# lazear/sage

Measured on NVIDIA H100. Metric: spectra/sec, higher is better.
Workload: dtype f32

## Files before the change

### sage_b200/csrc/kernels.cuh

```cuda
#pragma once
#include <type_traits>

#include "device_common.cuh"
#include "glibc_log.cuh"

#ifndef SAGE_B200_RARE_NOINLINE
#define SAGE_B200_RARE_NOINLINE 0
#endif
#if SAGE_B200_RARE_NOINLINE
#define SB_RARE __noinline__
#else
#define SB_RARE __forceinline__
#endif

namespace sb {

__device__ __forceinline__ uint32_t pep_partition(const DbView& db, float x, bool le) {
    uint32_t lo = 0, hi = db.n_pep;
    if (db.pep_lut != nullptr) {
        const float t = (x - db.plut_base) * db.plut_inv_w;
        if (t == t) {
            const int c = (int)fminf(fmaxf(floorf(t), -2.0f), (float)PEP_LUT_CELLS + 2.0f);
            lo = __ldg(db.pep_lut + min(max(c - 1, 0), (int)PEP_LUT_CELLS));
            hi = __ldg(db.pep_lut + min(max(c + 2, 0), (int)PEP_LUT_CELLS));
        }
    }
    const int kx = f32_key(x);
    while (lo < hi) {
        const uint32_t mid = lo + ((hi - lo) >> 1);
        const int k = f32_key(__ldg(db.pep_mono + mid));
        if (le ? k <= kx : k < kx) lo = mid + 1; else hi = mid;
    }
    return lo;
}

__global__ void k_setup_queries(DbView db, ScorerView sc, BatchView b, uint32_t* sort_key, uint32_t* sort_val) {
    __shared__ unsigned long long s_sum[4][8];
    const uint32_t s = blockIdx.x * blockDim.x + threadIdx.x;
    unsigned long long nq = 0, nwide = 0, maxpot = 0, npepq = 0, list_need = 0, ncta = 0;
    if (s < b.n) {
    const float pmz = b.prec_mz[s];
    const uint32_t known = b.prec_charge[s];
    const float mz = __fsub_rn(pmz, PROTON);
    const bool fold = sc.wide_window || !(known != 0 && !sc.override_charge);
    uint32_t c0 = fold ? sc.min_charge : known;
    uint32_t c1 = fold ? sc.max_charge : known;
    QueryDesc* out = b.queries + (size_t)s * sc.qmax;
    uint32_t qi = 0;
    for (uint32_t z = c0; z <= c1 && qi < sc.qmax; z++) {
        const float precursor_mass = __fmul_rn(mz, (float)z);
        Tol ptol = sc.precursor_tol;
        if (sc.wide_window) {
            float lo = -2.4f, hi = 2.4f;
            if (b.iso_lo != nullptr && !isnan(b.iso_lo[s]) && !isnan(b.iso_hi[s])) { lo = b.iso_lo[s]; hi = b.iso_hi[s]; }
            ptol.kind = 2;
            ptol.lo = __fmul_rn(lo, (float)z);
            ptol.hi = __fmul_rn(hi, (float)z);
        }
        const uint32_t mfc = max_fragment_charge(sc.max_fragment_charge_opt, z);
        for (uint32_t ii = 0; ii < sc.n_iso; ii++, qi++) {
            const int iso = (sc.min_iso != sc.max_iso) ? sc.min_iso + (int)ii : 0;
            const float qmass = __fsub_rn(precursor_mass, __fmul_rn((float)iso, NEUTRON));
            float plo, phi;
            tol_bounds(ptol, qmass, plo, phi);
            const uint32_t ppl = pep_partition(db, plo, false);
            const uint32_t left = ppl == 0 ? 0 : ppl - 1;
            const uint32_t right = max(left, pep_partition(db, phi, true));
            QueryDesc q;
            q.pre_lo = left;
            q.pre_hi = right;
            q.potential = right - left + 1;
            const bool lo_ok = left < db.n_pep && __ldg(db.pep_mono + left) >= plo;
            const bool hi_ok = right < db.n_pep && __ldg(db.pep_mono + right) <= phi;
            const long long elo = (long long)left + (lo_ok ? 0 : 1);
            const long long ehi = (long long)right - (hi_ok ? 0 : 1);
            if (ehi < elo) { q.eff_lo = 1; q.eff_hi = 0; } else { q.eff_lo = (uint32_t)elo; q.eff_hi = (uint32_t)ehi; }
            q.charge = (uint8_t)z;
            q.iso = (int8_t)iso;
            q.nfc = (uint8_t)(mfc - 1);
            q.mode = q.potential > NARROW_CAP ? 2 : ((db.pep_centric_ok && q.potential <= sc.pep_cap) ? 3 : (q.potential <= WARPQ_CAP ? 4 : 1));
            out[qi] = q;
            if (q.mode != 2 && q.potential > sc.kparam) list_need += q.potential;
            if (q.mode == 4) b.counters[C_COUNT + qi] = 1ull;
            ncta += (q.mode == 1 || q.mode == 3);
            nq++;
            if (q.mode == 2) {
                nwide++;
                QueryHits h0; h0.n = 0; h0.default_run = q.potential; h0.matched_peaks = 0; h0.scored_candidates = 0;
                b.hits[(size_t)s * sc.qmax + qi] = h0;
            }
            if (q.mode == 3) npepq++;
            if (q.potential > maxpot) maxpot = q.potential;
        }
    }
    for (; qi < sc.qmax; qi++) {
        QueryDesc q = {};
        out[qi] = q;
    }
    if (sort_key) { sort_key[s] = out[0].mode ? out[0].pre_lo : 0xFFFFFFFFu; sort_val[s] = s; }
    if (nwide) {
        unsigned long long w = atomicAdd(b.counters + C_WIDE, nwide);
        for (uint32_t j = 0; j < sc.qmax; j++)
            if (out[j].mode == 2) { if (w < b.wide_cap) b.wide_items[w] = s * sc.qmax + j; w++; }
    }
    if (ncta) {
        unsigned long long w = atomicAdd(b.counters + C_NCTA, ncta);
        for (uint32_t j = 0; j < sc.qmax; j++)
            if (out[j].mode == 1 || out[j].mode == 3) b.cta_items[w++] = s * sc.qmax + j;
    }
    for (uint32_t j = 0; j < sc.qmax; j++) {
        ReplaySlot rs; rs.off = 0; rs.item = s * sc.qmax + j; rs.n_list = 0; rs.state = 1; rs.k = 0;
        b.nslots[(size_t)s * sc.qmax + j] = rs;
    }
    }
    const uint32_t lane = threadIdx.x & 31, warp = threadIdx.x >> 5;
// ... 206 lines not shown
                        matched++;
                    }
                }
                if (stop) { e = cnt; break; }
            }
        }
        uint32_t pend = __ballot_sync(0xffffffffu, e < cnt);
        while (pend) {
            const int src = __ffs(pend) - 1;
            pend &= pend - 1;
            const uint32_t e0 = __shfl_sync(0xffffffffu, e, src);
            const float lo_s = __shfl_sync(0xffffffffu, flo, src), hi_s = __shfl_sync(0xffffffffu, fhi, src);
            for (uint32_t pos = e0; pos < cnt; pos += 32) {
                const uint32_t i = pos + lane;
                bool stop = i >= cnt;
                if (!stop) {
                    const float fmz = __ldg(mz + i);
                    const uint32_t pid = pep0 + __ldg(off + i);
                    stop = fmz > hi_s;
                    if (!stop && fmz >= lo_s) {
                        if (pid >= q.eff_lo && pid <= q.eff_hi) {
                            const uint32_t idx = pid - q.pre_lo;
                            atomicAdd(&cnt32[idx >> 1], 1u << ((idx & 1) * 16));
                            matched++;
                        }
                    }
                }
                if (__any_sync(0xffffffffu, stop)) break;
            }
        }
    }
}

__device__ __forceinline__ void narrow_cta_query(const DbView& db, const ScorerView& sc, const BatchView& b, uint32_t pmax, uint64_t* nlist, uint32_t item,
                                                 float* bounds_smem, const NarrowIndexView& nv) {
    __shared__ uint32_t cnt32[NARROW_CAP / 2 + 1];
    __shared__ uint32_t s_warp[40];
    ReplaySlot* const nslots = b.nslots;
    const uint32_t s = item / sc.qmax;
    const QueryDesc q = b.queries[item];
    const uint32_t tid = threadIdx.x, lane = tid & 31, warp = tid >> 5, nwarps = PRELIM_THREADS / 32;
    const uint32_t p0 = b.peak_off[s], np = b.peak_off[s + 1] - p0;
    const uint32_t nwords = (q.potential + 1) >> 1;
    for (uint32_t i = tid; i < nwords; i += PRELIM_THREADS) cnt32[i] = 0;
    __shared__ unsigned long long s_loff;
    if (tid == 0 && q.potential > sc.kparam) s_loff = atomicAdd(b.counters + C_NLIST, (unsigned long long)q.potential);

    const uint32_t nfc = q.nfc;
    const uint32_t ntask = np * nfc;
    uint32_t my_matched = 0, my_pages = 0, my_entries = 0;
    __shared__ LutParams s_lp[8];
    bool pep_path = q.mode == 3 && np > 0 && np < 65536 && nfc <= 8;
    float* const bnd = bounds_smem;
    uint16_t* const luts = reinterpret_cast<uint16_t*>(bounds_smem + 2 * (size_t)nfc * pmax);
    if (pep_path) {
        for (uint32_t t = tid; t < ntask; t += PRELIM_THREADS) {
            const uint32_t c = t / np, p = t - c * np;
            const float mass = __fmul_rn(__ldg(b.masses + p0 + p), (float)(c + 1));
            float flo, fhi;
            tol_bounds(sc.fragment_tol, mass, flo, fhi);
            bnd[(2 * c) * pmax + p] = flo;
            bnd[(2 * c + 1) * pmax + p] = fhi;
        }
        __syncthreads();
        bool bad = false;
        for (uint32_t t = tid; t < ntask; t += PRELIM_THREADS) {
            const uint32_t c = t / np, p = t - c * np;
            const float* lo_c = bnd + (2 * c) * pmax;
            const float* hi_c = lo_c + pmax;
            if (p > 0) bad |= !(lo_c[p] >= lo_c[p - 1]) || !(hi_c[p] >= hi_c[p - 1]);
            bad |= !(lo_c[p] == lo_c[p]) || !(hi_c[p] == hi_c[p]);
        }
        if (__syncthreads_or(bad)) {
            pep_path = false;
            if (tid == 0) atomicAdd(b.counters + C_PEPFALLBACK, 1ull);
        } else {
            for (uint32_t c = 0; c < nfc; c++) {
                const float* lo_c = bnd + (2 * c) * pmax;
                const float* hi_c = lo_c + pmax;
// ... 83 lines not shown
        for (uint32_t w = 0; w < nwarps; w++) { pages_total += s_red[1][w]; entries_total += s_red[2][w]; }
        atomicAdd(b.counters + C_TASKS, (unsigned long long)ntask);
        if (pages_total) atomicAdd(b.counters + C_PAGES, (unsigned long long)pages_total);
        if (entries_total) atomicAdd(b.counters + C_ENTRIES, (unsigned long long)entries_total);
        atomicAdd(b.counters + C_MATCHED, (unsigned long long)matched_total);
    }
    QueryHits* h = b.hits + item;
    if (matched_total == 0) {
        if (tid == 0) {
            h->n = 0; h->default_run = q.potential; h->matched_peaks = 0; h->scored_candidates = 0;
            nslots[item].off = 0; nslots[item].item = item; nslots[item].n_list = 0; nslots[item].state = 1; nslots[item].k = 0;
        }
        return;
    }
    const uint32_t n = q.potential, k = min(n, sc.kparam);
    auto cnt = [&](uint32_t i) -> uint32_t { return (cnt32[i >> 1] >> ((i & 1) * 16)) & 0xFFFFu; };
    ReplaySlot* slot = nslots + item;
    uint32_t nzc = 0;
    if (n <= k) {
        uint64_t* keys = b.hit_keys + (size_t)item * sc.kparam;
        for (uint32_t i = tid; i < n; i += PRELIM_THREADS) {
            const uint32_t c = cnt(i);
            nzc += c != 0;
            keys[i] = c ? prescore_key(c, q.pre_lo + i, q.charge, q.iso) : PRESCORE_DEFAULT;
        }
        const uint32_t nzt = block_sum_u32(nzc, s_warp);
        if (tid == 0) {
            h->n = n; h->default_run = 0; h->matched_peaks = matched_total; h->scored_candidates = nzt;
            slot->off = 0; slot->item = item; slot->n_list = 0; slot->state = 1; slot->k = k;
        }
        return;
    }
    const unsigned long long loff = s_loff;
    if (loff + n > b.nlist_cap) {
        if (tid == 0) {
            h->n = 0; h->default_run = q.potential; h->matched_peaks = 0; h->scored_candidates = 0;
            slot->off = 0; slot->item = item; slot->n_list = 0; slot->state = 1; slot->k = 0;
        }
        return;
    }
    uint64_t* list = nlist + loff;
    for (uint32_t i = tid; i < k; i += PRELIM_THREADS) {
        const uint32_t c = cnt(i);
        nzc += c != 0;
        list[i] = c ? prescore_key(c, q.pre_lo + i, q.charge, q.iso) : PRESCORE_DEFAULT;
    }
    uint32_t wbase = k;
    for (uint32_t base = k; base < n; base += PRELIM_THREADS) {
        const uint32_t i = base + tid;
        const uint32_t c = i < n ? cnt(i) : 0;
        nzc += c != 0;
        const uint32_t ball = __ballot_sync(0xffffffffu, c != 0);
        if (lane == 0) s_warp[warp] = __popc(ball);
        __syncthreads();
        uint32_t off = 0, total = 0;
        for (uint32_t w = 0; w < nwarps; w++) {
            const uint32_t x = s_warp[w];
            if (w < warp) off += x;
            total += x;
        }
        if (c) list[wbase + off + __popc(ball & ((1u << lane) - 1))] = prescore_key(c, q.pre_lo + i, q.charge, q.iso);
        wbase += total;
        __syncthreads();
    }
    const uint32_t nzt = block_sum_u32(nzc, s_warp);
    if (tid == 0) {
        h->n = k; h->default_run = 0; h->matched_peaks = matched_total; h->scored_candidates = nzt;
        slot->off = loff; slot->item = item; slot->n_list = wbase; slot->state = 0; slot->k = k;
    }
}

__global__ void __launch_bounds__(PRELIM_THREADS, PRELIM_CTAS) k_prelim_narrow(DbView db, ScorerView sc, BatchView b, uint32_t pmax, uint64_t* nlist, NarrowIndexView nv) {
    extern __shared__ float bounds_smem[];
    const uint32_t total = (uint32_t)min(b.counters[C_NCTA], (unsigned long long)b.n * sc.qmax);
    for (uint32_t i = blockIdx.x; i < total; i += gridDim.x) {
        narrow_cta_query(db, sc, b, pmax, nlist, b.cta_items[i], bounds_smem, nv);
        __syncthreads();
    }
}

template <bool BLK>
__global__ void __launch_bounds__(WARPQ_WARPS * 32, WARPQ_MIN_CTAS) k_prelim_narrow_warp(DbView db, ScorerView sc, BatchView b, uint64_t* nlist, uint32_t s_lo,
                                                                                                uint32_t s_hi, NarrowIndexView nv) {
    __shared__ uint32_t cnt_all[WARPQ_WARPS][WARPQ_CAP / 2];
    if (b.counters[C_COUNT + blockIdx.y] == 0ull) return;
    const uint32_t lane = threadIdx.x & 31, warp = threadIdx.x >> 5;
    const uint32_t pos = blockIdx.x * WARPQ_WARPS + warp;
    if (pos >= b.n) return;
    const uint32_t s = b.order ? b.order[pos] : pos;
    if (s < s_lo || s >= s_hi) return;
    const uint32_t item = s * sc.qmax + blockIdx.y;
    const QueryDesc q = b.queries[item];
    if (q.mode != 4) return;
    uint32_t* const cnt32 = cnt_all[warp];
    const uint32_t n = q.potential, k = min(n, sc.kparam);
    for (uint32_t i = lane; i < (n + 1) >> 1; i += 32) cnt32[i] = 0;
    unsigned long long loff = 0;
    if (n > k) {
        if (lane == 0) loff = atomicAdd(b.counters + C_NLIST, (unsigned long long)n);
        loff = __shfl_sync(0xffffffffu, loff, 0);
    }
    __syncwarp();
    const uint32_t p0 = b.peak_off[s], np = b.peak_off[s + 1] - p0;
    const uint32_t nfc = q.nfc, ntask = np * nfc;
    uint32_t matched = 0, pages = 0, entries = 0;
    const uint32_t blk0 = BLK ? q.pre_lo / nv.block : 0u, blk1 = BLK ? min(q.pre_hi, db.n_pep - 1) / nv.block : 0u;
    for (uint32_t t0 = 0; t0 < ntask; t0 += 32) {
        const uint32_t t = t0 + lane;
        const bool act = t < ntask;
        float flo = 0.0f, fhi = 0.0f;
        if (act) {
            const uint32_t p = t / nfc, fc = t - p * nfc + 1;
            const float mass = __fmul_rn(__ldg(b.masses + p0 + p), (float)fc);
            tol_bounds(sc.fragment_tol, mass, flo, fhi);
        }
        if (BLK) block_probe_warp(nv, q, blk0, blk1, act, flo, fhi, cnt32, matched);
        else if (act) index_probe(db, q, flo, fhi, cnt32, matched, pages, entries);
    }
    for (int o = 16; o > 0; o >>= 1) {
        matched += __shfl_xor_sync(0xffffffffu, matched, o);
        pages += __shfl_xor_sync(0xffffffffu, pages, o);
        entries += __shfl_xor_sync(0xffffffffu, entries, o);
    }
    __syncwarp();
    if (lane == 0) {
        atomicAdd(b.counters + C_TASKS, (unsigned long long)ntask);
        if (pages) atomicAdd(b.counters + C_PAGES, (unsigned long long)pages);
        if (entries) atomicAdd(b.counters + C_ENTRIES, (unsigned long long)entries);
        if (matched) atomicAdd(b.counters + C_MATCHED, (unsigned long long)matched);
    }
    QueryHits* h = b.hits + item;
    ReplaySlot* slot = b.nslots + item;
    if (matched == 0 || (n > k && loff + n > b.nlist_cap)) {
        if (lane == 0) { h->n = 0; h->default_run = n; h->matched_peaks = 0; h->scored_candidates = 0; }
        return;
    }
    auto cnt = [&](uint32_t i) -> uint32_t { return (cnt32[i >> 1] >> ((i & 1) * 16)) & 0xFFFFu; };
    uint32_t nzc = 0;
    uint64_t* dst = n <= k ? b.hit_keys + (size_t)item * sc.kparam : nlist + loff;
    for (uint32_t i = lane; i < k; i += 32) {
        const uint32_t c = cnt(i);
        nzc += c != 0;
        dst[i] = c ? prescore_key(c, q.pre_lo + i, q.charge, q.iso) : PRESCORE_DEFAULT;
    }
    uint32_t wbase = k;
    for (uint32_t base = k; base < n; base += 32) {
        const uint32_t i = base + lane;
        const uint32_t c = i < n ? cnt(i) : 0;
        nzc += c != 0;
        const uint32_t ball = __ballot_sync(0xffffffffu, c != 0);
        if (c) dst[wbase + __popc(ball & ((1u << lane) - 1))] = prescore_key(c, q.pre_lo + i, q.charge, q.iso);
        wbase += __popc(ball);
    }
    for (int o = 16; o > 0; o >>= 1) nzc += __shfl_xor_sync(0xffffffffu, nzc, o);
    if (lane == 0) {
        h->n = k; h->default_run = 0; h->matched_peaks = matched; h->scored_candidates = nzc;
        if (n > k) { slot->off = loff; slot->n_list = wbase; slot->state = 0; slot->k = k; }
    }
}

#ifndef SAGE_B200_WIDE_THREADS
#define SAGE_B200_WIDE_THREADS 512
#endif
#ifndef SAGE_B200_WIDE_TILE
#define SAGE_B200_WIDE_TILE (32 * 1024)
#endif
#ifndef SAGE_B200_WIDE_CTAS
#define SAGE_B200_WIDE_CTAS 2
#endif
constexpr int WIDE_THREADS = SAGE_B200_WIDE_THREADS;
constexpr int WIDE_CTAS = SAGE_B200_WIDE_CTAS;
constexpr bool WIDE_SMALL = WIDE_CTAS > 1;
constexpr uint32_t WIDE_TILE = SAGE_B200_WIDE_TILE;
constexpr uint32_t WIDE_VMAX = WIDE_SMALL ? 1024 : 2048;
constexpr uint32_t WIDE_TCACHE = WIDE_SMALL ? 1024 : 2048;
constexpr uint32_t WIDE_LMAX = 12288;
constexpr uint32_t WIDE_HLEV = 64;
typedef ReplaySlot WideSlot;
struct WideRange { uint64_t start; uint32_t len; float flo, fhi; };

constexpr uint32_t WIDE_VCAP = WIDE_SMALL ? 512 : 1024;
constexpr uint32_t WIDE_BT = 16;
struct WideSlow {
    uint32_t cur[WIDE_VMAX];
// ... 567 lines not shown
    const QueryDesc q = b.queries[item];
    const uint32_t s = item / sc.qmax;
    const uint32_t p0 = b.peak_off[s], np = b.peak_off[s + 1] - p0;
    const uint32_t nfc = q.nfc, ntask = np * nfc;
    if (ntask > WIDE_TMAX) return;
    unsigned long long pages = 0, entries = 0;
    for (uint32_t t = lane; t < ntask; t += 32) {
        const uint32_t p = t / nfc, fc = t - p * nfc + 1;
        const float mass = __fmul_rn(__ldg(b.masses + p0 + p), (float)fc);
        float flo, fhi;
        tol_bounds(sc.fragment_tol, mass, flo, fhi);
        uint32_t bl, br;
        bucket_range(db, flo, fhi, bl, br);
        for (uint32_t page = bl; page < br; page++) {
            const uint64_t pbase = (uint64_t)page * db.bucket_size;
            const uint32_t pn = (uint32_t)(min(pbase + db.bucket_size, db.n_frag) - pbase);
            const uint32_t st = page_lower_bound_dir(db, page, db.frag + pbase, pn, q.pre_lo);
            const uint32_t en = page_lower_bound_dir(db, page, db.frag + pbase, pn, q.pre_hi + 1);
            entries += en - (st == 0 ? 0 : st - 1);
            pages++;
        }
    }
    for (int o = 16; o > 0; o >>= 1) {
        pages += __shfl_down_sync(0xffffffffu, pages, o);
        entries += __shfl_down_sync(0xffffffffu, entries, o);
    }
    if (lane == 0) {
        if (pages) atomicAdd(b.counters + C_PAGES, pages);
        if (entries) atomicAdd(b.counters + C_ENTRIES, entries);
    }
}

constexpr int REPLAY_THREADS = 128;
template <bool COMPACT>
__global__ void __launch_bounds__(REPLAY_THREADS) k_replay(ScorerView sc, BatchView b, const uint64_t* lists, const ReplaySlot* slots, uint32_t n_slots,
                                                           const unsigned long long* n_slots_dev, uint32_t n_spectra) {
    typedef typename std::conditional<COMPACT, uint32_t, uint64_t>::type key_t;
    extern __shared__ __align__(8) unsigned char rheap_raw[];
    key_t* const rheap = reinterpret_cast<key_t*>(rheap_raw);
    uint32_t slot = blockIdx.x * REPLAY_THREADS + threadIdx.x;
    if (n_slots_dev != nullptr) n_slots = (uint32_t)min((unsigned long long)n_slots, *n_slots_dev);
    if (slot >= n_slots) return;
    if (n_spectra) { const uint32_t pos = slot % n_spectra; slot = (b.order ? b.order[pos] : pos) * sc.qmax + slot / n_spectra; }
    const ReplaySlot ws = slots[slot];
    if (ws.state != 0) return;
    const uint64_t* list = lists + ws.off;
    const uint32_t k = ws.k, tid = threadIdx.x;
    uint32_t pre_lo = 0, q_charge = 0;
    int q_iso = 0;
    if (COMPACT) { const QueryDesc q = b.queries[ws.item]; pre_lo = q.pre_lo; q_charge = q.charge; q_iso = q.iso; }
    auto pack = [&](uint64_t k64) -> key_t {
        if (!COMPACT) return (key_t)k64;
        return (key_t)(key_peptide(k64) == 0xFFFFFFFFu ? 0x0000FFFFu : ((key_matched(k64) << 16) | (key_peptide(k64) - pre_lo)));
    };
    auto unpack = [&](key_t kk) -> uint64_t {
        if (!COMPACT) return (uint64_t)kk;
        const uint32_t v = (uint32_t)kk;
        return v == 0x0000FFFFu ? PRESCORE_DEFAULT : prescore_key(v >> 16, pre_lo + (v & 0xFFFFu), q_charge, q_iso);
    };
    auto H = [&](uint32_t i) -> key_t& { return rheap[i * REPLAY_THREADS + tid]; };
    auto sift = [&](uint32_t index, key_t val) {
        for (;;) {
            const uint32_t l = index * 2 + 1;
            if (l >= k) break;
            uint32_t c = l;
            key_t cv = H(l);
            if (l + 1 < k) { const key_t cr = H(l + 1); if (cr < cv) { cv = cr; c = l + 1; } }
            if (!(cv < val)) break;
            H(index) = cv;
            index = c;
        }
        H(index) = val;
    };
    for (uint32_t i = 0; i < k; i++) H(i) = pack(__ldg(list + i));
    for (uint32_t i = k / 2; i-- > 0;) sift(i, H(i));
    key_t root = H(0);
    uint64_t nxt = k < ws.n_list ? __ldg(list + k) : 0;
    for (uint32_t j = k; j < ws.n_list; j++) {
        const key_t kq = pack(nxt);
        if (j + 1 < ws.n_list) nxt = __ldg(list + j + 1);
        if (kq > root) { sift(0, kq); root = H(0); }
    }
    uint64_t* keys = b.hit_keys + (size_t)ws.item * sc.kparam;
    for (uint32_t i = 0; i < k; i++) keys[i] = unpack(H(i));
}

struct ScoreRec {
    double hyperscore;
    uint32_t peptide;
    uint32_t matched_b, matched_y;
    float summed_b, summed_y;
    uint32_t longest_b, longest_y;
    float ppm_difference;
    uint32_t charge;
    int iso;
    uint32_t valid;
    uint32_t plen;
};

__device__ SB_RARE int select_most_intense_peak(const float* masses, const float* intens, uint32_t n, float center, const Tol& tol) {
    float lo, hi;
    tol_bounds(tol, center, lo, hi);
    lo = __fadd_rn(lo, 0.0f);
    hi = __fadd_rn(hi, 0.0f);
    const int klo = f32_key(lo), khi = f32_key(hi);
    uint32_t i, j;
    binary_search_slice(n, [&](uint32_t k) { return f32_key(masses[k]) < klo; }, [&](uint32_t k) { return f32_key(masses[k]) <= khi; }, i, j);
    int best = -1;
    float max_int = 0.0f;
    for (uint32_t idx = i; idx < j; idx++) {
        const float m = masses[idx];
        if (m >= lo && m <= hi) {
            const float it = intens[idx];
            if (it >= max_int) { max_int = it; best = (int)idx; }
        }
    }
    return best;
// ... 1350 lines not shown
```

### sage_b200/csrc/sage_b200.cu

```cuda
#include <cub/device/device_radix_sort.cuh>
#include <cub/device/device_scan.cuh>
#include <cub/device/device_select.cuh>
#include <cub/device/device_reduce.cuh>
#include <cuda_runtime.h>
#include <thrust/iterator/counting_iterator.h>

#include <pthread.h>
#include <sched.h>

#include <algorithm>
#include <atomic>
#include <cctype>
#include <cmath>
#include <cstdarg>
#include <cstdio>
#include <cstdlib>
#include <cstring>
#include <chrono>
#include <condition_variable>
#include <memory>
#include <mutex>
#include <thread>
#include <string>
#include <vector>
// ... 1147 lines not shown

    CUDA_TRY(cudaStreamWaitEvent(st, S->lanes[(&L - S->lanes) ^ 1].ev[4], 0));
    CUDA_TRY(cudaStreamWaitEvent(st, L.ev_small, 0));
    CUDA_TRY(cudaEventRecord(L.ev[6], st));
    CUDA_TRY(cudaMemsetAsync(L.d_counters.p, 0, 8 * (C_COUNT + (size_t)sv.qmax), st));
    const bool annotate = sv.annotate && S->frag_dst != nullptr;
    if (annotate) {
        if ((rc = L.d_frags.reserve(S->frag_cap * sizeof(sage_b200_fragment) + 64))) return rc;
        unsigned long long* hbase = (unsigned long long*)L.h_counters.p + C_COUNT + 1;
        *hbase = S->frag_used;
        CUDA_TRY(cudaMemcpyAsync(L.d_counters.as<unsigned long long>() + C_FRAGS, hbase, 8, cudaMemcpyHostToDevice, st));
    }
    ScorerView svq = sv;
    uint32_t mfc = sv.max_fragment_charge_opt >= 0 ? std::min<uint32_t>(C.zmax, (uint32_t)(sv.max_fragment_charge_opt + 1) & 0xFF) : C.zmax;
    if (mfc < 2) mfc = 2;
    size_t pep_smem = (size_t)(mfc - 1) * (2 * (size_t)C.pmax * sizeof(float) + 2 * LUT_CELLS * sizeof(uint16_t));
    if (mfc - 1 > 8) pep_smem = 200 * 1024;
    if (pep_smem > 96 * 1024) { svq.pep_cap = 0; pep_smem = 0; }
    if (svq.pep_cap == 0) pep_smem = 0;
    uint32_t *sk_in = nullptr, *sk_out = nullptr, *sv_in = nullptr, *sv_out = nullptr;
    int sort_bits = 1;
    while (sort_bits < 32 && (db->v.n_pep >> sort_bits)) sort_bits++;
    const int sort_lo = std::max(0, sort_bits - 16);
    size_t sort_tmp = 0;
    if (S->sort_spectra && n > 1) {
        if ((rc = L.d_sort.reserve(16 * (size_t)n))) return rc;
        sk_in = L.d_sort.as<uint32_t>(); sk_out = sk_in + n; sv_in = sk_out + n; sv_out = sv_in + n;
        CUDA_TRY(cub::DeviceRadixSort::SortPairs(nullptr, sort_tmp, sk_in, sk_out, sv_in, sv_out, (int)n, sort_lo, sort_bits, st));
        if ((rc = L.d_sorttmp.reserve(sort_tmp + 16))) return rc;
    }
    C.nlist_cap = std::max<uint64_t>(C.force_nlist, (uint64_t)std::ceil(S->nlist_per_spectrum * (double)n) + 4096);
    C.wide_cap = (uint32_t)std::min<uint64_t>(C.nitems, std::max<uint64_t>(C.force_wide, S->wide_per_spectrum > 0.0
                                                                               ? (uint64_t)std::ceil(S->wide_per_spectrum * 1.1 * (double)n) + 64 : 0));
    if ((rc = L.d_nlist.reserve(8 * (C.nlist_cap + 16)))) return rc;
    if ((rc = L.d_nslots.reserve(C.nitems * sizeof(ReplaySlot)))) return rc;
    if (C.wide_cap) {
        if ((rc = L.d_witems.reserve(4 * (size_t)C.wide_cap))) return rc;
        if ((rc = L.d_wlist.reserve((size_t)C.wide_cap * WIDE_LMAX * 8))) return rc;
        if ((rc = L.d_wslots.reserve((size_t)C.wide_cap * sizeof(WideSlot)))) return rc;
    }
    if ((rc = L.d_citems.reserve(4 * C.nitems))) return rc;
    bv.cta_items = L.d_citems.as<uint32_t>();
    bv.nslots = L.d_nslots.as<ReplaySlot>();
    bv.wide_items = L.d_witems.as<uint32_t>();
    bv.wide_cap = C.wide_cap;
    bv.nlist_cap = C.nlist_cap;
    k_setup_queries<<<(n + 127) / 128, 128, 0, st>>>(db->v, svq, bv, sk_in, sv_in);
    CUDA_TRY(cudaGetLastError());
    if (sk_in) {
        CUDA_TRY(cub::DeviceRadixSort::SortPairs(L.d_sorttmp.p, sort_tmp, sk_in, sk_out, sv_in, sv_out, (int)n, sort_lo, sort_bits, st));
        bv.order = sv_out;
    }
    CUDA_TRY(cudaEventRecord(L.ev[2], st));
    if (C.nparts <= 1) CUDA_TRY(cudaStreamWaitEvent(st, L.ev_masses, 0));
    uint64_t launches = 1;

    const size_t rsm = (size_t)sv.kparam * REPLAY_THREADS * 8;
    const float ptol_span = std::max(std::fabs(sv.precursor_tol.lo), std::fabs(sv.precursor_tol.hi));
    const bool narrow_tol = ptol_span <= (sv.precursor_tol.kind == 0 ? 2000.0f : sv.precursor_tol.kind == 1 ? 0.2f : 5.0f);
    NarrowIndexView nv{};
    if (S->narrow_index && !sv.wide_window && narrow_tol) {
        if (S->narrow_block == 0 && (rc = narrow_block_for(S))) return rc;
        nv = db_narrow_index(db, S->narrow_block ? S->narrow_block : S->narrow_block_auto, S->narrow_block != 0);
    }
    for (uint32_t q = 0; q < C.nparts; q++) {
        if (C.nparts > 1) CUDA_TRY(cudaStreamWaitEvent(st, L.ev_part[q], 0));
        const dim3 wgrid((n + WARPQ_WARPS - 1) / WARPQ_WARPS, sv.qmax);
        if (nv.mz != nullptr) k_prelim_narrow_warp<true><<<wgrid, WARPQ_WARPS * 32, 0, st>>>(db->v, svq, bv, L.d_nlist.as<uint64_t>(), C.part_lo[q], C.part_lo[q + 1], nv);
        else k_prelim_narrow_warp<false><<<wgrid, WARPQ_WARPS * 32, 0, st>>>(db->v, svq, bv, L.d_nlist.as<uint64_t>(), C.part_lo[q], C.part_lo[q + 1], nv);
        CUDA_TRY(cudaGetLastError());
        launches += q > 0;
    }
    if (C.nparts > 1) CUDA_TRY(cudaStreamWaitEvent(st, L.ev_masses, 0));
    k_prelim_narrow<<<(unsigned)std::min<uint64_t>(C.nitems, (uint64_t)db->sm_count * PRELIM_CTAS), PRELIM_THREADS, pep_smem, st>>>(db->v, svq, bv, C.pmax, L.d_nlist.as<uint64_t>(),
                                                                                                                         S->narrow_cta ? nv : NarrowIndexView{});
    CUDA_TRY(cudaGetLastError());
    CUDA_TRY(cudaEventRecord(L.ev[8], st));
    k_replay<true><<<(unsigned)((C.nitems + REPLAY_THREADS - 1) / REPLAY_THREADS), REPLAY_THREADS, rsm / 2, st>>>(sv, bv, L.d_nlist.as<uint64_t>(), L.d_nslots.as<ReplaySlot>(),
                                                                                                                 (uint32_t)C.nitems, nullptr, n);
    CUDA_TRY(cudaGetLastError());
    launches += 3;
    if (C.wide_cap) {
        const int ctas = (int)std::min<uint64_t>((uint64_t)db->sm_count * WIDE_CTAS, C.wide_cap);
        const WideIndexView wv = db_wide_index(db, sv.wide_tile);
        k_prelim_wide<<<ctas, WIDE_THREADS, sizeof(WideSmem), st>>>(db->v, sv, bv, (uint32_t)C.nitems, L.d_wlist.as<uint64_t>(), L.d_wslots.as<WideSlot>(), wv);
        CUDA_TRY(cudaGetLastError());
        if (wv.frag != nullptr) {
            k_wide_account<<<(C.wide_cap + 7) / 8, 256, 0, st>>>(db->v, sv, bv);
            CUDA_TRY(cudaGetLastError());
            launches++;
        }
        k_replay<false><<<(unsigned)((C.wide_cap + REPLAY_THREADS - 1) / REPLAY_THREADS), REPLAY_THREADS, rsm, st>>>(
            sv, bv, L.d_wlist.as<uint64_t>(), L.d_wslots.as<WideSlot>(), C.wide_cap, L.d_counters.as<unsigned long long>() + C_WIDE, 0u);
        CUDA_TRY(cudaGetLastError());
        launches += 2;
    }
    CUDA_TRY(cudaEventRecord(L.ev[3], st));

    if ((rc = lane_join_stager(L))) return rc;
    CUDA_TRY(cudaStreamWaitEvent(st, L.ev_intens, 0));
    const bool split = S->score_split && !sv.chimera && !annotate && !dbg && S->quick_mode == 0;
    if (split) {
        C.hits_cap = std::max<uint64_t>(C.force_hits, (uint64_t)std::ceil((S->hits_per_spectrum > 0.0 ? S->hits_per_spectrum : 4096.0) * (double)n) + 65536);
        if ((rc = L.d_cand.reserve((size_t)n * sv.kparam * sizeof(CandOut)))) return rc;
        if ((rc = L.d_meta.reserve((size_t)n * sizeof(SpecMeta)))) return rc;
        if ((rc = L.d_recs.reserve((size_t)n * sv.kparam * sizeof(ScoreRec)))) return rc;
        if ((rc = L.d_hkey.reserve((size_t)n * sv.kparam * 8))) return rc;
        if ((rc = L.d_emit.reserve((size_t)n * sv.report_psms * 4 + 16))) return rc;
        if ((rc = L.d_hitk.reserve(2 * C.hits_cap + 16))) return rc;
        if ((rc = L.d_hiti.reserve(4 * C.hits_cap + 16))) return rc;
        if ((rc = L.d_hitt.reserve(4 * C.hits_cap + 16))) return rc;
        SplitOut so{};
// ... 1748 lines not shown
        FDR_TRY(cudaGetLastError());
    }
    k_rt_align<<<(unsigned)((n_files + 127) / 128), 128, 0, st>>>(d_mat, d_mean, n_rows, n_files, d_maxrt, d_align);
    FDR_TRY(cudaGetLastError());
    float* d_aligned = d_out[0];
    k_rt_aligned<<<g, 256, 0, st>>>(d_rows, d_file, n, d_align, d_aligned);
    FDR_TRY(cudaGetLastError());
    FDR_TRY(cudaEventRecord(ev[2], st));

    if (int rc = rt_model<0>(st, A, fma, pk, d_rows, n, d_train, n_train, d_aligned, d_aligned, d_out[1], d_out[2], &out->rt_fitted, &out->rt_r2,
                             &out->rt_eps, out->rt_beta))
        return rc;
    FDR_TRY(cudaEventRecord(ev[3], st));
    if (int rc = rt_model<1>(st, A, fma, pk, d_rows, n, d_train, n_train, nullptr, d_aligned, d_out[3], d_out[4], &out->ims_fitted, &out->ims_r2,
                             &out->ims_eps, out->ims_beta))
        return rc;
    FDR_TRY(cudaEventRecord(ev[4], st));

    float* dst[5] = {out->aligned_rt, out->predicted_rt, out->delta_rt_model, out->predicted_ims, out->delta_ims_model};
    for (int c = 0; c < 5; c++) FDR_TRY(cudaMemcpyAsync(dst[c], d_out[c], 4 * n, cudaMemcpyDeviceToHost, st));
    if (out->spectrum_q) FDR_TRY(cudaMemcpyAsync(out->spectrum_q, d_q, 4 * n, cudaMemcpyDeviceToHost, st));
    FDR_TRY(cudaMemcpyAsync(out->alignments, d_align, sizeof(sage_b200_alignment) * n_files, cudaMemcpyDeviceToHost, st));
    FDR_TRY(cudaStreamSynchronize(st));
    out->training_rows = n_train;
    out->aligned_peptides = n_rows;
    float* ms[4] = {&out->ms_sort_q, &out->ms_alignment, &out->ms_rt_model, &out->ms_ims_model};
    for (int i = 0; i < 4; i++) FDR_TRY(cudaEventElapsedTime(ms[i], ev[i], ev[i + 1]));
    FDR_TRY(cudaEventElapsedTime(&out->ms_total, ev[0], ev[4]));
    return 0;
}
#undef FDR_TRY

#if SAGE_B200_PHASE_CLOCKS
extern "C" int sage_b200_debug_phase_cycles(unsigned long long* out16, int reset) {
    if (out16) CUDA_TRY(cudaMemcpyFromSymbol(out16, g_phase, sizeof(unsigned long long) * 16));
    if (reset) { unsigned long long z[16] = {0}; CUDA_TRY(cudaMemcpyToSymbol(g_phase, z, sizeof z)); }
    return 0;
}
#endif
```

Before: 24.73 million.

## Store narrow candidate lists as compact 32-bit keys and restructure replay heap

Narrow prelim kernels now write 32-bit compact keys (matched<<16 | offset) into the candidate list instead of 64-bit prescore keys. List reservations are padded to multiples of four so replay can fetch four keys per vector load. The replay kernel loads each heap cooperatively across the warp, keeps the top seven heap nodes in registers, uses a two-level sift, and writes outputs coalesced per warp. This halves list memory traffic and cuts shared-memory work per replacement, at the cost of more registers and more code complexity. It also adds optional phase-clock instrumentation.

Result: faster. 25.37 million (median of 6 runs) (+2.6%).

```diff
diff --git a/sage_b200/csrc/kernels.cuh b/sage_b200/csrc/kernels.cuh
--- a/sage_b200/csrc/kernels.cuh
+++ b/sage_b200/csrc/kernels.cuh
@@ -33,6 +33,10 @@
     }
     return lo;
 }
+
+constexpr uint32_t LIST_KEY_DEFAULT = 0x0000FFFFu;
+__device__ __forceinline__ uint32_t list_key(uint32_t matched, uint32_t i) { return matched ? (matched << 16) | i : LIST_KEY_DEFAULT; }
+__host__ __device__ __forceinline__ uint32_t list_reserve(uint32_t potential) { return (potential + 3u) & ~3u; }
 
 __global__ void k_setup_queries(DbView db, ScorerView sc, BatchView b, uint32_t* sort_key, uint32_t* sort_val) {
     __shared__ unsigned long long s_sum[4][8];
@@ -80,7 +84,7 @@
             q.nfc = (uint8_t)(mfc - 1);
             q.mode = q.potential > NARROW_CAP ? 2 : ((db.pep_centric_ok && q.potential <= sc.pep_cap) ? 3 : (q.potential <= WARPQ_CAP ? 4 : 1));
             out[qi] = q;
-            if (q.mode != 2 && q.potential > sc.kparam) list_need += q.potential;
+            if (q.mode != 2 && q.potential > sc.kparam) list_need += list_reserve(q.potential);
             if (q.mode == 4) b.counters[C_COUNT + qi] = 1ull;
             ncta += (q.mode == 1 || q.mode == 3);
             nq++;
@@ -353,7 +357,7 @@
     }
 }
 
-__device__ __forceinline__ void narrow_cta_query(const DbView& db, const ScorerView& sc, const BatchView& b, uint32_t pmax, uint64_t* nlist, uint32_t item,
+__device__ __forceinline__ void narrow_cta_query(const DbView& db, const ScorerView& sc, const BatchView& b, uint32_t pmax, uint32_t* nlist, uint32_t item,
                                                  float* bounds_smem, const NarrowIndexView& nv) {
     __shared__ uint32_t cnt32[NARROW_CAP / 2 + 1];
     __shared__ uint32_t s_warp[40];
@@ -365,7 +369,7 @@
     const uint32_t nwords = (q.potential + 1) >> 1;
     for (uint32_t i = tid; i < nwords; i += PRELIM_THREADS) cnt32[i] = 0;
     __shared__ unsigned long long s_loff;
-    if (tid == 0 && q.potential > sc.kparam) s_loff = atomicAdd(b.counters + C_NLIST, (unsigned long long)q.potential);
+    if (tid == 0 && q.potential > sc.kparam) s_loff = atomicAdd(b.counters + C_NLIST, (unsigned long long)list_reserve(q.potential));
 
     const uint32_t nfc = q.nfc;
     const uint32_t ntask = np * nfc;
@@ -515,18 +519,18 @@
         return;
     }
     const unsigned long long loff = s_loff;
-    if (loff + n > b.nlist_cap) {
+    if (loff + list_reserve(n) > b.nlist_cap) {
         if (tid == 0) {
             h->n = 0; h->default_run = q.potential; h->matched_peaks = 0; h->scored_candidates = 0;
             slot->off = 0; slot->item = item; slot->n_list = 0; slot->state = 1; slot->k = 0;
         }
         return;
     }
-    uint64_t* list = nlist + loff;
+    uint32_t* list = nlist + loff;
     for (uint32_t i = tid; i < k; i += PRELIM_THREADS) {
         const uint32_t c = cnt(i);
         nzc += c != 0;
-        list[i] = c ? prescore_key(c, q.pre_lo + i, q.charge, q.iso) : PRESCORE_DEFAULT;
+        list[i] = list_key(c, i);
     }
     uint32_t wbase = k;
     for (uint32_t base = k; base < n; base += PRELIM_THREADS) {
@@ -542,7 +546,7 @@
             if (w < warp) off += x;
             total += x;
         }
-        if (c) list[wbase + off + __popc(ball & ((1u << lane) - 1))] = prescore_key(c, q.pre_lo + i, q.charge, q.iso);
+        if (c) list[wbase + off + __popc(ball & ((1u << lane) - 1))] = list_key(c, i);
         wbase += total;
         __syncthreads();
     }
@@ -553,7 +557,7 @@
     }
 }
 
-__global__ void __launch_bounds__(PRELIM_THREADS, PRELIM_CTAS) k_prelim_narrow(DbView db, ScorerView sc, BatchView b, uint32_t pmax, uint64_t* nlist, NarrowIndexView nv) {
+__global__ void __launch_bounds__(PRELIM_THREADS, PRELIM_CTAS) k_prelim_narrow(DbView db, ScorerView sc, BatchView b, uint32_t pmax, uint32_t* nlist, NarrowIndexView nv) {
     extern __shared__ float bounds_smem[];
     const uint32_t total = (uint32_t)min(b.counters[C_NCTA], (unsigned long long)b.n * sc.qmax);
     for (uint32_t i = blockIdx.x; i < total; i += gridDim.x) {
@@ -563,7 +567,7 @@
 }
 
 template <bool BLK>
-__global__ void __launch_bounds__(WARPQ_WARPS * 32, WARPQ_MIN_CTAS) k_prelim_narrow_warp(DbView db, ScorerView sc, BatchView b, uint64_t* nlist, uint32_t s_lo,
+__global__ void __launch_bounds__(WARPQ_WARPS * 32, WARPQ_MIN_CTAS) k_prelim_narrow_warp(DbView db, ScorerView sc, BatchView b, uint32_t* nlist, uint32_t s_lo,
                                                                                                 uint32_t s_hi, NarrowIndexView nv) {
     __shared__ uint32_t cnt_all[WARPQ_WARPS][WARPQ_CAP / 2];
     if (b.counters[C_COUNT + blockIdx.y] == 0ull) return;
@@ -580,7 +584,7 @@
     for (uint32_t i = lane; i < (n + 1) >> 1; i += 32) cnt32[i] = 0;
     unsigned long long loff = 0;
     if (n > k) {
-        if (lane == 0) loff = atomicAdd(b.counters + C_NLIST, (unsigned long long)n);
+        if (lane == 0) loff = atomicAdd(b.counters + C_NLIST, (unsigned long long)list_reserve(n));
         loff = __shfl_sync(0xffffffffu, loff, 0);
     }
     __syncwarp();
@@ -614,17 +618,26 @@
     }
     QueryHits* h = b.hits + item;
     ReplaySlot* slot = b.nslots + item;
-    if (matched == 0 || (n > k && loff + n > b.nlist_cap)) {
+    if (matched == 0 || (n > k && loff + list_reserve(n) > b.nlist_cap)) {
         if (lane == 0) { h->n = 0; h->default_run = n; h->matched_peaks = 0; h->scored_candidates = 0; }
         return;
     }
     auto cnt = [&](uint32_t i) -> uint32_t { return (cnt32[i >> 1] >> ((i & 1) * 16)) & 0xFFFFu; };
     uint32_t nzc = 0;
-    uint64_t* dst = n <= k ? b.hit_keys + (size_t)item * sc.kparam : nlist + loff;
-    for (uint32_t i = lane; i < k; i += 32) {
-        const uint32_t c = cnt(i);
-        nzc += c != 0;
-        dst[i] = c ? prescore_key(c, q.pre_lo + i, q.charge, q.iso) : PRESCORE_DEFAULT;
+    uint32_t* const list = nlist + loff;
+    if (n <= k) {
+        uint64_t* keys = b.hit_keys + (size_t)item * sc.kparam;
+        for (uint32_t i = lane; i < k; i += 32) {
+            const uint32_t c = cnt(i);
+            nzc += c != 0;
+            keys[i] = c ? prescore_key(c, q.pre_lo + i, q.charge, q.iso) : PRESCORE_DEFAULT;
+        }
+    } else {
+        for (uint32_t i = lane; i < k; i += 32) {
+            const uint32_t c = cnt(i);
+            nzc += c != 0;
+            list[i] = list_key(c, i);
+        }
     }
     uint32_t wbase = k;
     for (uint32_t base = k; base < n; base += 32) {
@@ -632,7 +645,7 @@
         const uint32_t c = i < n ? cnt(i) : 0;
         nzc += c != 0;
         const uint32_t ball = __ballot_sync(0xffffffffu, c != 0);
-        if (c) dst[wbase + __popc(ball & ((1u << lane) - 1))] = prescore_key(c, q.pre_lo + i, q.charge, q.iso);
+        if (c) list[wbase + __popc(ball & ((1u << lane) - 1))] = list_key(c, i);
         wbase += __popc(ball);
     }
     for (int o = 16; o > 0; o >>= 1) nzc += __shfl_xor_sync(0xffffffffu, nzc, o);
@@ -1266,57 +1279,165 @@
 }
 
 constexpr int REPLAY_THREADS = 128;
+constexpr int REPLAY_STRIDE = REPLAY_THREADS;
+constexpr uint32_t REPLAY_BATCH = 8;
+static_assert(REPLAY_BATCH % 4 == 0, "narrow lists are fetched four keys per load");
+
+#if SAGE_B200_PHASE_CLOCKS
+__device__ unsigned long long g_replay_phase[16];
+#endif
+
 template <bool COMPACT>
-__global__ void __launch_bounds__(REPLAY_THREADS) k_replay(ScorerView sc, BatchView b, const uint64_t* lists, const ReplaySlot* slots, uint32_t n_slots,
-                                                           const unsigned long long* n_slots_dev, uint32_t n_spectra) {
+__global__ void __launch_bounds__(REPLAY_THREADS) k_replay(ScorerView sc, BatchView b, const typename std::conditional<COMPACT, uint32_t, uint64_t>::type* lists,
+                                                           const ReplaySlot* slots, uint32_t n_slots, const unsigned long long* n_slots_dev,
+                                                           uint32_t n_spectra) {
     typedef typename std::conditional<COMPACT, uint32_t, uint64_t>::type key_t;
     extern __shared__ __align__(8) unsigned char rheap_raw[];
     key_t* const rheap = reinterpret_cast<key_t*>(rheap_raw);
-    uint32_t slot = blockIdx.x * REPLAY_THREADS + threadIdx.x;
-    if (n_slots_dev != nullptr) n_slots = (uint32_t)min((unsigned long long)n_slots, *n_slots_dev);
-    if (slot >= n_slots) return;
-    if (n_spectra) { const uint32_t pos = slot % n_spectra; slot = (b.order ? b.order[pos] : pos) * sc.qmax + slot / n_spectra; }
-    const ReplaySlot ws = slots[slot];
-    if (ws.state != 0) return;
-    const uint64_t* list = lists + ws.off;
-    const uint32_t k = ws.k, tid = threadIdx.x;
+    const uint32_t tid = threadIdx.x, lane = tid & 31, col0 = tid & ~31u;
+    uint32_t slot = blockIdx.x * REPLAY_THREADS + tid;
+    ReplaySlot ws; ws.off = 0; ws.item = 0; ws.n_list = 0; ws.state = 1; ws.k = 0;
     uint32_t pre_lo = 0, q_charge = 0;
     int q_iso = 0;
-    if (COMPACT) { const QueryDesc q = b.queries[ws.item]; pre_lo = q.pre_lo; q_charge = q.charge; q_iso = q.iso; }
-    auto pack = [&](uint64_t k64) -> key_t {
-        if (!COMPACT) return (key_t)k64;
-        return (key_t)(key_peptide(k64) == 0xFFFFFFFFu ? 0x0000FFFFu : ((key_matched(k64) << 16) | (key_peptide(k64) - pre_lo)));
-    };
-    auto unpack = [&](key_t kk) -> uint64_t {
-        if (!COMPACT) return (uint64_t)kk;
-        const uint32_t v = (uint32_t)kk;
-        return v == 0x0000FFFFu ? PRESCORE_DEFAULT : prescore_key(v >> 16, pre_lo + (v & 0xFFFFu), q_charge, q_iso);
-    };
-    auto H = [&](uint32_t i) -> key_t& { return rheap[i * REPLAY_THREADS + tid]; };
-    auto sift = [&](uint32_t index, key_t val) {
-        for (;;) {
-            const uint32_t l = index * 2 + 1;
-            if (l >= k) break;
-            uint32_t c = l;
-            key_t cv = H(l);
-            if (l + 1 < k) { const key_t cr = H(l + 1); if (cr < cv) { cv = cr; c = l + 1; } }
-            if (!(cv < val)) break;
-            H(index) = cv;
-            index = c;
-        }
-        H(index) = val;
-    };
-    for (uint32_t i = 0; i < k; i++) H(i) = pack(__ldg(list + i));
-    for (uint32_t i = k / 2; i-- > 0;) sift(i, H(i));
-    key_t root = H(0);
-    uint64_t nxt = k < ws.n_list ? __ldg(list + k) : 0;
-    for (uint32_t j = k; j < ws.n_list; j++) {
-        const key_t kq = pack(nxt);
-        if (j + 1 < ws.n_list) nxt = __ldg(list + j + 1);
-        if (kq > root) { sift(0, kq); root = H(0); }
-    }
-    uint64_t* keys = b.hit_keys + (size_t)ws.item * sc.kparam;
-    for (uint32_t i = 0; i < k; i++) keys[i] = unpack(H(i));
+    if (n_slots_dev != nullptr) n_slots = (uint32_t)min((unsigned long long)n_slots, *n_slots_dev);
+    if (slot < n_slots) {
+        if (n_spectra) { const uint32_t pos = slot % n_spectra; slot = (b.order ? b.order[pos] : pos) * sc.qmax + slot / n_spectra; }
+        ws = slots[slot];
+        if (COMPACT && ws.state == 0) { const QueryDesc q = b.queries[ws.item]; pre_lo = q.pre_lo; q_charge = q.charge; q_iso = q.iso; }
+    }
+    const uint32_t k = ws.state == 0 ? ws.k : 0, n_list = ws.n_list;
+    const key_t* const list = lists + ws.off;
+    const uint32_t owners = __ballot_sync(0xffffffffu, k != 0);
+    if (owners == 0) return;
+#if SAGE_B200_PHASE_CLOCKS
+    const long long t0 = clock64();
+#endif
+    for (uint32_t m = owners; m; m &= m - 1) {
+        const int o = __ffs(m) - 1;
+        const uint32_t ko = __shfl_sync(0xffffffffu, k, o);
+        const key_t* const lo = lists + __shfl_sync(0xffffffffu, ws.off, o);
+        for (uint32_t i = lane; i < ko; i += 32) rheap[i * REPLAY_STRIDE + col0 + o] = __ldg(lo + i);
+    }
+    __syncwarp();
+#if SAGE_B200_PHASE_CLOCKS
+    long long t1 = t0, t2 = t0;
+#endif
+    if (k != 0) {
+        auto H = [&](uint32_t i) -> key_t& { return rheap[i * REPLAY_STRIDE + tid]; };
+        auto sift = [&](uint32_t index, key_t val) {
+            for (;;) {
+                const uint32_t l = index * 2 + 1;
+                if (l >= k) break;
+                uint32_t c = l;
+                key_t cv = H(l);
+                if (l + 1 < k) { const key_t cr = H(l + 1); if (cr < cv) { cv = cr; c = l + 1; } }
+                if (!(cv < val)) break;
+                H(index) = cv;
+                index = c;
+            }
+            H(index) = val;
+        };
+        for (uint32_t i = k / 2; i-- > 0;) sift(i, H(i));
+#if SAGE_B200_PHASE_CLOCKS
+        t1 = clock64();
+#endif
+        key_t h0 = H(0), h1 = H(1), h2 = H(2), h3 = H(3), h4 = H(4), h5 = H(5), h6 = H(6);
+        auto sift_pairs = [&](uint32_t index, key_t val) {
+            const key_t none = ~(key_t)0;
+            for (;;) {
+                const uint32_t l = index * 2 + 1, g = l * 2 + 1;
+                if (l >= k) break;
+                const key_t cl = H(l), cr = l + 1 < k ? H(l + 1) : none;
+                const key_t g0 = g < k ? H(g) : none, g1 = g + 1 < k ? H(g + 1) : none, g2 = g + 2 < k ? H(g + 2) : none, g3 = g + 3 < k ? H(g + 3) : none;
+                const bool r = cr < cl;
+                const key_t cv = r ? cr : cl;
+                if (!(cv < val)) break;
+                H(index) = cv;
+                index = l + (uint32_t)r;
+                const key_t ga = r ? g2 : g0, gb = r ? g3 : g1;
+                const bool rr = gb < ga;
+                const key_t gv = rr ? gb : ga;
+                if (!(gv < val)) break;
+                H(index) = gv;
+                index = index * 2 + 1 + (uint32_t)rr;
+            }
+            H(index) = val;
+        };
+        auto replace_root = [&](key_t val) {
+            const bool r0 = h2 < h1;
+            const key_t c0 = r0 ? h2 : h1;
+            if (!(c0 < val)) { h0 = val; return; }
+            h0 = c0;
+            const key_t a = r0 ? h5 : h3, bb = r0 ? h6 : h4;
+            const bool r1 = bb < a;
+            const key_t c1 = r1 ? bb : a;
+            if (!(c1 < val)) { if (r0) h2 = val; else h1 = val; return; }
+            if (r0) h2 = c1; else h1 = c1;
+            const uint32_t at = 3 + 2 * (uint32_t)r0 + (uint32_t)r1, l = 2 * at + 1;
+            const key_t x = H(l), y = H(l + 1);
+            const bool r2 = y < x;
+            const key_t c2 = r2 ? y : x;
+            const bool stay = !(c2 < val);
+            const key_t put = stay ? val : c2;
+            if (r0) { if (r1) h6 = put; else h5 = put; } else { if (r1) h4 = put; else h3 = put; }
+            if (!stay) sift_pairs(l + (uint32_t)r2, val);
+        };
+        if (COMPACT) {
+            const uint4* const l4 = reinterpret_cast<const uint4*>(list);
+            for (uint32_t j0 = k & ~3u; j0 < n_list; j0 += REPLAY_BATCH) {
+                uint4 v4[REPLAY_BATCH / 4];
+#pragma unroll
+                for (uint32_t e = 0; e < REPLAY_BATCH / 4; e++) v4[e] = j0 + 4 * e < n_list ? __ldg(l4 + (j0 >> 2) + e) : make_uint4(0, 0, 0, 0);
+#pragma unroll
+                for (uint32_t e = 0; e < REPLAY_BATCH; e++) {
+                    const uint4 v = v4[e >> 2];
+                    const uint32_t kq = (e & 3) == 0 ? v.x : (e & 3) == 1 ? v.y : (e & 3) == 2 ? v.z : v.w;
+                    const uint32_t j = j0 + e;
+                    if (j >= k && j < n_list && kq > h0) replace_root((key_t)kq);
+                }
+            }
+        } else {
+            for (uint32_t j0 = k; j0 < n_list; j0 += REPLAY_BATCH) {
+                key_t v[REPLAY_BATCH];
+#pragma unroll
+                for (uint32_t e = 0; e < REPLAY_BATCH; e++) v[e] = j0 + e < n_list ? __ldg(list + j0 + e) : (key_t)0;
+#pragma unroll
+                for (uint32_t e = 0; e < REPLAY_BATCH; e++)
+                    if (j0 + e < n_list && v[e] > h0) replace_root(v[e]);
+            }
+        }
+        H(0) = h0; H(1) = h1; H(2) = h2; H(3) = h3; H(4) = h4; H(5) = h5; H(6) = h6;
+#if SAGE_B200_PHASE_CLOCKS
+        t2 = clock64();
+#endif
+    }
+    __syncwarp();
+    for (uint32_t m = owners; m; m &= m - 1) {
+        const int o = __ffs(m) - 1;
+        const uint32_t ko = __shfl_sync(0xffffffffu, k, o);
+        uint64_t* const keys = b.hit_keys + (size_t)__shfl_sync(0xffffffffu, ws.item, o) * sc.kparam;
+        const uint32_t o_lo = __shfl_sync(0xffffffffu, pre_lo, o), o_charge = __shfl_sync(0xffffffffu, q_charge, o);
+        const int o_iso = __shfl_sync(0xffffffffu, q_iso, o);
+        for (uint32_t i = lane; i < ko; i += 32) {
+            const key_t kk = rheap[i * REPLAY_STRIDE + col0 + o];
+            if (COMPACT) {
+                const uint32_t v = (uint32_t)kk;
+                keys[i] = v == LIST_KEY_DEFAULT ? PRESCORE_DEFAULT : prescore_key(v >> 16, o_lo + (v & 0xFFFFu), o_charge, o_iso);
+            } else {
+                keys[i] = (uint64_t)kk;
+            }
+        }
+    }
+#if SAGE_B200_PHASE_CLOCKS
+    if (k != 0) {
+        const long long t3 = clock64();
+        const unsigned long long d[3] = {(unsigned long long)(t1 - t0), (unsigned long long)(t2 - t1), (unsigned long long)(t3 - t2)};
+        for (int i = 0; i < 3; i++) { atomicAdd(&g_replay_phase[i], d[i]); atomicMax(&g_replay_phase[3 + i], d[i]); }
+        atomicAdd(&g_replay_phase[6], 1ull);
+        atomicMax(&g_replay_phase[7], (unsigned long long)(n_list - k));
+        atomicAdd(&g_replay_phase[8 + min(7, 32 - __clz(n_list - k))], 1ull);
+    }
+#endif
 }
 
 struct ScoreRec {
diff --git a/sage_b200/csrc/sage_b200.cu b/sage_b200/csrc/sage_b200.cu
--- a/sage_b200/csrc/sage_b200.cu
+++ b/sage_b200/csrc/sage_b200.cu
@@ -1203,7 +1203,7 @@
     C.nlist_cap = std::max<uint64_t>(C.force_nlist, (uint64_t)std::ceil(S->nlist_per_spectrum * (double)n) + 4096);
     C.wide_cap = (uint32_t)std::min<uint64_t>(C.nitems, std::max<uint64_t>(C.force_wide, S->wide_per_spectrum > 0.0
                                                                                ? (uint64_t)std::ceil(S->wide_per_spectrum * 1.1 * (double)n) + 64 : 0));
-    if ((rc = L.d_nlist.reserve(8 * (C.nlist_cap + 16)))) return rc;
+    if ((rc = L.d_nlist.reserve(4 * (C.nlist_cap + 16)))) return rc;
     if ((rc = L.d_nslots.reserve(C.nitems * sizeof(ReplaySlot)))) return rc;
     if (C.wide_cap) {
         if ((rc = L.d_witems.reserve(4 * (size_t)C.wide_cap))) return rc;
@@ -1226,7 +1226,7 @@
     if (C.nparts <= 1) CUDA_TRY(cudaStreamWaitEvent(st, L.ev_masses, 0));
     uint64_t launches = 1;
 
-    const size_t rsm = (size_t)sv.kparam * REPLAY_THREADS * 8;
+    const size_t rsm = (size_t)sv.kparam * REPLAY_STRIDE * 8;
     const float ptol_span = std::max(std::fabs(sv.precursor_tol.lo), std::fabs(sv.precursor_tol.hi));
     const bool narrow_tol = ptol_span <= (sv.precursor_tol.kind == 0 ? 2000.0f : sv.precursor_tol.kind == 1 ? 0.2f : 5.0f);
     NarrowIndexView nv{};
@@ -1234,21 +1234,22 @@
         if (S->narrow_block == 0 && (rc = narrow_block_for(S))) return rc;
         nv = db_narrow_index(db, S->narrow_block ? S->narrow_block : S->narrow_block_auto, S->narrow_block != 0);
     }
+    uint32_t* const nlist = L.d_nlist.as<uint32_t>();
     for (uint32_t q = 0; q < C.nparts; q++) {
         if (C.nparts > 1) CUDA_TRY(cudaStreamWaitEvent(st, L.ev_part[q], 0));
         const dim3 wgrid((n + WARPQ_WARPS - 1) / WARPQ_WARPS, sv.qmax);
-        if (nv.mz != nullptr) k_prelim_narrow_warp<true><<<wgrid, WARPQ_WARPS * 32, 0, st>>>(db->v, svq, bv, L.d_nlist.as<uint64_t>(), C.part_lo[q], C.part_lo[q + 1], nv);
-        else k_prelim_narrow_warp<false><<<wgrid, WARPQ_WARPS * 32, 0, st>>>(db->v, svq, bv, L.d_nlist.as<uint64_t>(), C.part_lo[q], C.part_lo[q + 1], nv);
+        if (nv.mz != nullptr) k_prelim_narrow_warp<true><<<wgrid, WARPQ_WARPS * 32, 0, st>>>(db->v, svq, bv, nlist, C.part_lo[q], C.part_lo[q + 1], nv);
+        else k_prelim_narrow_warp<false><<<wgrid, WARPQ_WARPS * 32, 0, st>>>(db->v, svq, bv, nlist, C.part_lo[q], C.part_lo[q + 1], nv);
         CUDA_TRY(cudaGetLastError());
         launches += q > 0;
     }
     if (C.nparts > 1) CUDA_TRY(cudaStreamWaitEvent(st, L.ev_masses, 0));
-    k_prelim_narrow<<<(unsigned)std::min<uint64_t>(C.nitems, (uint64_t)db->sm_count * PRELIM_CTAS), PRELIM_THREADS, pep_smem, st>>>(db->v, svq, bv, C.pmax, L.d_nlist.as<uint64_t>(),
+    k_prelim_narrow<<<(unsigned)std::min<uint64_t>(C.nitems, (uint64_t)db->sm_count * PRELIM_CTAS), PRELIM_THREADS, pep_smem, st>>>(db->v, svq, bv, C.pmax, nlist,
                                                                                                                          S->narrow_cta ? nv : NarrowIndexView{});
     CUDA_TRY(cudaGetLastError());
     CUDA_TRY(cudaEventRecord(L.ev[8], st));
-    k_replay<true><<<(unsigned)((C.nitems + REPLAY_THREADS - 1) / REPLAY_THREADS), REPLAY_THREADS, rsm / 2, st>>>(sv, bv, L.d_nlist.as<uint64_t>(), L.d_nslots.as<ReplaySlot>(),
-                                                                                                                 (uint32_t)C.nitems, nullptr, n);
+    k_replay<true><<<(unsigned)((C.nitems + REPLAY_THREADS - 1) / REPLAY_THREADS), REPLAY_THREADS, rsm / 2, st>>>(sv, bv, nlist, L.d_nslots.as<ReplaySlot>(), (uint32_t)C.nitems,
+                                                                                                                 nullptr, n);
     CUDA_TRY(cudaGetLastError());
     launches += 3;
     if (C.wide_cap) {
@@ -3063,6 +3064,11 @@
 #undef FDR_TRY
 
 #if SAGE_B200_PHASE_CLOCKS
+extern "C" int sage_b200_debug_replay_cycles(unsigned long long* out16, int reset) {
+    if (out16) CUDA_TRY(cudaMemcpyFromSymbol(out16, g_replay_phase, sizeof(unsigned long long) * 16));
+    if (reset) { unsigned long long z[16] = {0}; CUDA_TRY(cudaMemcpyToSymbol(g_replay_phase, z, sizeof z)); }
+    return 0;
+}
 extern "C" int sage_b200_debug_phase_cycles(unsigned long long* out16, int reset) {
     if (out16) CUDA_TRY(cudaMemcpyFromSymbol(out16, g_phase, sizeof(unsigned long long) * 16));
     if (reset) { unsigned long long z[16] = {0}; CUDA_TRY(cudaMemcpyToSymbol(g_phase, z, sizeof z)); }
```
